# AgamChopra/TorchRegister

Hardware: AMD Instinct MI355X
Metric: registration iterations/sec (3D 256^3 fp32, affine+NCC) (higher is better)
Workload: dtype f32; 1 GPU; 3D 256^3 fp32 affine+NCC, 8 independent pairs per GPU (BASELINE.json configs[3] share of one GPU), ADAM on theta; pairs_per_gpu=8, pairs_total=8, loss=NCC(alpha=100), optimizer=adam, preconditioning=100 untimed iterations before the warm-up (clock settling); value_cold has none, parallelism=1 x independent shards, no collective

## Files before the change

include/trx.h:

```cpp
#ifndef TRX_H
#define TRX_H

#include <stddef.h>
#include <stdint.h>

#ifdef __cplusplus
extern "C" {
#endif

#define TRX_VERSION 240
#define TRX_PSTRIDE 12

typedef enum {
    TRX_OK = 0,
    TRX_ERR_ARG = -1,
    TRX_ERR_NDIM = -2,
    TRX_ERR_WORKSPACE = -3,
    TRX_ERR_HIP = -4,
    TRX_ERR_CAPACITY = -5
} trx_status;

#define TRX_FLAG_GATHER_PATH 1u
#define TRX_FLAG_SINGLE_GEOM 2u
#define TRX_FLAG_TWO_PASS_FLOW 4u
#define TRX_FLAG_DEEP_TILE 8u
#define TRX_FLAG_SAVE_LAST 256u
#define TRX_FLAG_NEAREST 128u
#define TRX_FLAG_NO_ZSTREAM 32u
#define TRX_FLAG_ZSTREAM 64u
#define TRX_FLAG_NO_EFT 512u
#define TRX_FLAG_EFT 1024u
#define TRX_FLAG_ZS_FUSED 2048u
#define TRX_FLAG_WALK_DOWN 8192u
#define TRX_FLAG_NO_PINGPONG 16384u
#define TRX_FLAG_NO_ZS_FLAT 4096u
#define TRX_FLAG_ONE_KERNEL 32768u
#define TRX_FLAG_NO_CARRY 65536u
#define TRX_FLAG_NO_ROT_DEEP_TILE 16u

typedef struct {
    const float *moving;
    const float *target;
    size_t moving_stride;
    size_t target_stride;
    int ndim, B, D, H, W;
    const float *xn, *yn, *zn;
    unsigned flags;
} trx_volumes;

typedef struct {
    float w_mse, w_ncc, ncc_alpha, w_ssd, ssd_alpha;
} trx_loss_cfg;
// ... 150 lines not shown
```

torchregister_amd/_lib.py:

```python
import ctypes
import os

import torch

_HERE = os.path.dirname(os.path.abspath(__file__))
LIB_PATH = os.path.join(_HERE, "lib", "libtrx.so")

PSTRIDE = 12
OPT_SGD, OPT_ADAM = 0, 1
PARAM_AFFINE, PARAM_RIGID = 0, 1
FLAG_GATHER_PATH, FLAG_SINGLE_GEOM, FLAG_TWO_PASS_FLOW, FLAG_DEEP_TILE, FLAG_NO_ROT_DEEP_TILE, FLAG_NO_ZSTREAM, FLAG_ZSTREAM, FLAG_NEAREST, FLAG_SAVE_LAST = 1, 2, 4, 8, 16, 32, 64, 128, 256
FLAG_NO_EFT, FLAG_EFT = 512, 1024
FLAG_WALK_DOWN, FLAG_NO_PINGPONG = 8192, 16384
FLAG_NO_ZS_FLAT = 4096
FLAG_ONE_KERNEL = 32768
FLAG_NO_CARRY = 65536
FLAG_ZS_FUSED = 2048

c_float_p = ctypes.POINTER(ctypes.c_float)
c_int_p = ctypes.POINTER(ctypes.c_int)


class TrxError(RuntimeError):
    pass


class Volumes(ctypes.Structure):
    _fields_ = [("moving", ctypes.c_void_p), ("target", ctypes.c_void_p),
                ("moving_stride", ctypes.c_size_t), ("target_stride", ctypes.c_size_t),
                ("ndim", ctypes.c_int), ("B", ctypes.c_int), ("D", ctypes.c_int), ("H", ctypes.c_int), ("W", ctypes.c_int),
                ("xn", ctypes.c_void_p), ("yn", ctypes.c_void_p), ("zn", ctypes.c_void_p), ("flags", ctypes.c_uint)]
# ... 123 lines not shown
```

torchregister_amd/csrc/affine.hip:

```cpp
#ifdef TRX_DEV
#include <cstdlib>
#endif
#include "trx_dev.h"

#include "trx_common.h"

namespace trx {

struct AffineGeom {
    int TX, TY, logTX, RPT, nxseg, nychunk, nblk;
};

static AffineGeom affine_geom(const trx_volumes &v, int target_blocks_total)
{
    AffineGeom g;
    int tx = 16, l = 4;
    while (tx < v.W && tx < TRX_BLOCK) { tx <<= 1; l++; }
    g.TX = tx; g.logTX = l; g.TY = TRX_BLOCK / tx;
    g.nxseg = (v.W + tx - 1) / tx;
    long rows = (long)v.D * v.H * g.nxseg * v.B;
    long rpt = rows / ((long)g.TY * target_blocks_total);
    if (rpt < 1) rpt = 1;
    if (rpt > 64) rpt = 64;
    g.RPT = (int)rpt;
// ... 1204 lines not shown
    zs_step_main<MODE, 0>(vol, theta, zg, zgf, partials, rows_used, stride, 0, ring);
}

template <int MODE>
__global__ __launch_bounds__(ZS64::Threads, TRX_ZS_MIN_WAVES) void affine_zs_one_kernel(trx_volumes vol, const float *__restrict__ theta, ZGeom zg, ZGeom zgf, float *__restrict__ partials,
                                                                                        int *__restrict__ rows_used, int stride, TileGeom tgR)
{
    constexpr int kAllocZ = ZSF::Alloc > ZS64::Alloc ? ZSF::Alloc : ZS64::Alloc;
    constexpr int kAlloc = GeomR::BoxAlloc > kAllocZ ? GeomR::BoxAlloc : kAllocZ;
    __shared__ __attribute__((aligned(16))) float ring[kAlloc];
    zs_step_main<MODE, 1>(vol, theta, zg, zgf, partials, rows_used, stride, tgR.blocks_per_pair, ring);
}

template <int MODE>
__global__ __launch_bounds__(ECfg::Threads, 4) void affine_eft_step_kernel(trx_volumes vol, const float *__restrict__ theta, TileGeom tg, float *__restrict__ partials,
                                                                           int *__restrict__ rows_used, int stride, int with_d, int with_rd, int zs_planes_)
{
    const bool zs_first = zs_planes_ < 0;
    const int zs_planes = zs_first ? 0 : zs_planes_;
    __shared__ __attribute__((aligned(16))) float lds[ECfg::Alloc];
    __shared__ int s_ef[64];
    const int wave = trx_wave_index(), lane = trx_lane_id();
    const float fD = (float)vol.D, fH = (float)vol.H, fW = (float)vol.W;
    if (stride < 0) {
        if ((int)blockIdx.x >= tg.blocks_per_pair) return;
        const int b = blockIdx.y;
        const float *th = theta + (size_t)b * TRX_PSTRIDE;
        bool take = __builtin_amdgcn_readfirstlane((int)eft_wants(dual_choice(th, fD, fH, fW, with_d != 0, with_rd != 0, zs_planes), th, fD, fH, fW)) &&
                    __builtin_amdgcn_readfirstlane((int)ef_candidate(th, fD, fH, fW));
        if (take) {
            const EfMap m = ef_map(th, fD, fH, fW);
// ... 22 lines not shown
    const bool flat = stride >= 0;
#if TRX_EF_STAMP
    if (flat && wave == 0 && lane == 0) { for (int k = 1; k < 8; k++) trx_ef_blocks[blockIdx.x * 8 + k] = 0; trx_ef_blocks[blockIdx.x * 8] = __builtin_amdgcn_s_memrealtime(); }
#endif
    int pre = 0, total = 1;
    if (flat) {
    if (zs_first && __builtin_amdgcn_readfirstlane(rows_used[vol.B]) == 0) return;
    unsigned long long zs_mask = 0;
    if (zs_first) zs_mask = (unsigned long long)(unsigned)__builtin_amdgcn_readfirstlane(rows_used[vol.B + 1]) | ((unsigned long long)(unsigned)__builtin_amdgcn_readfirstlane(rows_used[vol.B + 2]) << 32);
    const bool free_l = lane < vol.B && !((zs_mask >> lane) & 1ull);
    const bool cand_l = free_l && eft_wants(dual_choice(theta + (size_t)lane * TRX_PSTRIDE, fD, fH, fW, with_d != 0, with_rd != 0, zs_planes),
                                                  theta + (size_t)lane * TRX_PSTRIDE, fD, fH, fW) &&
                        ef_candidate(theta + (size_t)lane * TRX_PSTRIDE, fD, fH, fW);
    const unsigned long long cand = __builtin_amdgcn_ballot_w64(cand_l);
    unsigned long long fit = 0;
    if (cand) {
        if (wave == 0) s_ef[lane] = 0;
        __syncthreads();
        unsigned long long rest = cand;
        for (int k = 0; rest; k++) {
            const int pb = __builtin_ctzll(rest);
            rest &= rest - 1;
            if ((k & (ECfg::Waves - 1)) != wave) continue;
            const EfMap m = ef_map(theta + (size_t)pb * TRX_PSTRIDE, fD, fH, fW);
            const EfDims d = ef_dims(m);
            const int g = ef_plan_granules_wave(m, d, lane);
            if (lane == 0) s_ef[pb] = (d.ok && g > 0 && g <= ECfg::GCap) ? 1 : 0;
        }
        __syncthreads();
        fit = __builtin_amdgcn_ballot_w64(s_ef[lane] != 0) & cand;
    }
// ... 23 lines not shown
        if (flat) {
            if (tickets) {
                int ord = qk / per_pair_q;
                const int j = qk - ord * per_pair_q;
                if (vol.flags & TRX_FLAG_WALK_DOWN) ord = total / tg.blocks_per_pair - 1 - ord;
                pair = __builtin_popcountll(__builtin_amdgcn_ballot_w64(pre <= ord * tg.blocks_per_pair));
                v = q + 8 * j;
            } else {
                pair = __builtin_popcountll(__builtin_amdgcn_ballot_w64(pre <= item));
                const int off = pair > 0 ? __builtin_amdgcn_readlane(pre, pair - 1) : 0;
                v = (item - off + 104 * pair) % tg.blocks_per_pair;
            }
        }
        v = __builtin_amdgcn_readfirstlane(v); pair = __builtin_amdgcn_readfirstlane(pair);
        if (item != it0) __syncthreads();
        eft_body<MODE>(vol, theta, tg, partials, lds, v, pair, rows_stride, wave, pr, pair != planned);
        planned = pair;
#if TRX_EF_STAMP
        if (flat && wave == 0 && lane == 0) { trx_ef_blocks[blockIdx.x * 8 + 1 + min((item - it0) / it_step, 5)] = __builtin_amdgcn_s_memrealtime(); }
#endif
        if (tickets) {
            if (wave == 0 && lane == 0) {
                const int first = (int)gridDim.x >> 3;
                int nq = blockIdx.x & 7, k = qlen;
                for (int t = 0; t < 8 && k >= qlen; t++) {
                    nq = ((int)blockIdx.x + t) & 7;
                    k = __hip_atomic_fetch_add(rows_used + vol.B + 3 + nq, 1, __ATOMIC_RELAXED, __HIP_MEMORY_SCOPE_AGENT) + first;
                }
                s_ef[63] = k < qlen ? ((nq << 24) | k) : -1;
            }
            __syncthreads();
            const int nx = __builtin_amdgcn_readfirstlane(s_ef[63]);
            if (nx < 0) break;
            q = nx >> 24; qk = nx & 0xffffff;
        }
    }
}

#pragma clang diagnostic pop


__global__ void fill_tables_kernel(float *__restrict__ tab, int W, int H, int D)
{
    const int i = blockIdx.x * blockDim.x + threadIdx.x;
    if (i < W) tab[i] = (float)(2 * i + 1) / (float)W - 1.0f;
    if (i < H) tab[W + i] = (float)(2 * i + 1) / (float)H - 1.0f;
    if (i < D) tab[W + H + i] = (float)(2 * i + 1) / (float)D - 1.0f;
}

struct LossCoef {
    double total, mse, ncc, ssd, cy, cw, c0;
};

// ... 206 lines not shown
    }
    if (i < NT) {
        if (theta_out) theta_out[i] = th_new;
        if (theta_lds) theta_lds[i] = th_new;
    }
}

constexpr int kCarryStride = 64;
constexpr int kCarryTheta = 0, kCarryParam = 12, kCarryM = 24, kCarryV = 36, kCarryStep = 48;

template <int ND>
__global__ __launch_bounds__(TRX_FIN_THREADS) void affine_finalize_kernel(const float *__restrict__ partials, int nblk,
                                                                          double nvox, int D, int H, int W,
                                                                          trx_loss_cfg lc, trx_opt_cfg oc,
                                                                          trx_affine_state st, const int *__restrict__ rows_used = nullptr, int mse_rows = 0,
                                                                          const float *__restrict__ state_in = nullptr)
{
    constexpr int NP = np_full(ND);
    constexpr int NT = ND * (ND + 1);
    constexpr int NPOSE = (ND == 3) ? 6 : 3;
    __shared__ double S[64];
    const int b = blockIdx.x;
    __shared__ double sh_dth[NT];
    __shared__ float sh_pose[NPOSE];
    const int i = threadIdx.x;
    const bool rigid = st.mode == TRX_PARAM_RIGID;
    float *param = st.param + (size_t)b * TRX_PSTRIDE;
    float *theta = st.theta + (size_t)b * TRX_PSTRIDE;
    FinRegs<ND> r;
    if (i < 64) {
        if (state_in) {
            const float *sb = state_in + (size_t)b * kCarryStride;
            r = fin_load<ND>(sb + kCarryParam, sb + kCarryTheta, sb + kCarryM, sb + kCarryV, reinterpret_cast<const int *>(sb + kCarryStep), st.best_loss + b,
                             oc.kind == TRX_OPT_ADAM, rigid, i);
        } else {
            r = fin_load<ND>(param, theta, st.adam_m ? st.adam_m + (size_t)b * TRX_PSTRIDE : nullptr, st.adam_v ? st.adam_v + (size_t)b * TRX_PSTRIDE : nullptr, st.step + b,
                             st.best_loss + b, oc.kind == TRX_OPT_ADAM, rigid, i);
        }
    }
    {
        int rows = nblk;
        if (rows_used) rows = min(abs(rows_used[b]) & kRowsMask, nblk);
        if (ND == 3 && mse_rows) reduce_partials<kNpMse>(partials + (size_t)b * nblk * kNpMse, rows, S);
        else reduce_partials<NP>(partials + (size_t)b * nblk * NP, rows, S);
    }
    if (i >= 64) return;
    fin_apply<ND>(S, r, b, i, nvox, D, H, W, lc, oc, st, mse_rows, param, theta, st.adam_m ? st.adam_m + (size_t)b * TRX_PSTRIDE : nullptr,
                  st.adam_v ? st.adam_v + (size_t)b * TRX_PSTRIDE : nullptr, st.step + b, true, nullptr, sh_dth, sh_pose);
}

template <int MODE>
__device__ __forceinline__ void carry_prologue(CarryKPtr c, int b, bool designated, int D, int H, int W, float *scratch, float *s_th, int wave, int lane)
{
    constexpr int NP = (MODE == 4) ? kNpMse : np_full(3);
    constexpr int NT = 12;
    const float *prev = c->prev_partials;
    const float *sp = c->state_prev;
    float *sn = c->state_next;
    const trx_affine_state st = {c->st.mode, c->st.param, c->st.theta, c->st.adam_m, c->st.adam_v, c->st.best_theta, c->st.best_loss, c->st.best_idx, c->st.losses,
                                 c->st.losses_capacity, c->st.step, c->st.grad};
    const trx_opt_cfg oc = {c->oc.kind, c->oc.lr, c->oc.beta1, c->oc.beta2, c->oc.eps};
    const bool adam = oc.kind == TRX_OPT_ADAM, rigid = st.mode == TRX_PARAM_RIGID;
    const float *src_theta = sp ? sp + (size_t)b * kCarryStride + kCarryTheta : st.theta + (size_t)b * TRX_PSTRIDE;
// ... 362 lines not shown
    int dev = 0, cus = 0;
    if (hipGetDevice(&dev) != hipSuccess || hipDeviceGetAttribute(&cus, hipDeviceAttributeMultiprocessorCount, dev) != hipSuccess || cus <= 0)
        return TRX_PERSISTENT_BLOCKS;
    return 2 * cus;
}

enum DualInstance { kTwoBody = 3, kFiveBody = 0, kBehindZs = 4, kCarry = 6 };
template <int W> struct Which { static constexpr int value = W; };
struct F1Plan {
    TileGeom ta, tr, td, trd, tef;
    ZGeom zg, zgf;
    int rows, slots;
    bool flat;
    bool zs_first, one_kernel;
    int eft;
    DualInstance dual;
};

static F1Plan f1_candidates(const trx_volumes &v)
{
    F1Plan p = F1Plan{};
    p.ta = tile_geom<GeomA>(v); p.tr = tile_geom<GeomR>(v); p.td = tile_geom<GeomD>(v); p.trd = p.tef = tile_geom<GeomRD>(v);
    if (zs_shape_ok<ZS64>(v)) p.zg = zs_geom<ZS64>(v);
    if (zs_shape_ok<ZSF>(v)) p.zgf = zs_geom<ZSF>(v);
    return p;
}

static int f1_rows(const F1Plan &p)
{
    return max(max(max(p.ta.blocks_per_pair, p.tr.blocks_per_pair), max(p.td.blocks_per_pair, p.trd.blocks_per_pair)),
// ... 19 lines not shown
    else if (p.zg.blocks_per_pair > 0 && !(v.flags & TRX_FLAG_ZSTREAM)) {
        const long zb = (long)p.zg.blocks_per_pair * v.B;
        if (zb < TRX_ZS_MIN_BLOCKS || p.zg.planes_per_seg < TRX_ZS_MIN_PLANES) p.zg = ZGeom{};
        else if (zb > slots / 2 && zb < slots && (long)p.ta.blocks_per_pair * v.B <= slots) p.zg = ZGeom{};
    }
    if (p.zg.blocks_per_pair == 0) p.zgf = ZGeom{};
    const TileGeom tef = p.tef;
    p.tef = TileGeom{};
    p.rows = f1_rows(p);
    p.flat = v.B <= 64 && (long)p.rows * v.B >= 2 * slots;
    const bool eft_sizes = (long)v.H * v.W * 4 < (1l << 24) && (size_t)v.D * v.H * v.W < ((size_t)1 << 29);
    if (tef.tiles_per_seg <= 64 && eft_sizes && !(v.flags & TRX_FLAG_NO_EFT) && (p.flat || (v.flags & TRX_FLAG_EFT))) {
        p.tef = tef;
        p.eft = tef.blocks_per_pair;
        p.rows = f1_rows(p);
    }
    if (v.flags & TRX_FLAG_NO_ZS_FLAT) p.zgf = ZGeom{};
    p.zs_first = p.flat && p.zg.blocks_per_pair > 0 && !(v.flags & TRX_FLAG_ZS_FUSED);
    p.one_kernel = p.zs_first && (v.flags & TRX_FLAG_ONE_KERNEL);
    const bool two_body = !p.flat && p.td.blocks_per_pair == 0 && p.trd.blocks_per_pair == 0 && p.zg.blocks_per_pair == 0 && p.eft == 0;
    p.dual = p.zs_first ? kBehindZs : !two_body ? kFiveBody : carry ? kCarry : kTwoBody;
    return p;
}

struct AffineWs {
    size_t rows, off_tab, off_rows_used, off_part2, off_rows_used2, off_carry, bytes;
};
static AffineWs affine_ws(const trx_volumes &v)
{
    AffineWs w;
    AffineGeom g = affine_geom(v, kTargetBlocks);
    w.rows = (size_t)g.nblk;
    if (v.ndim == 3) w.rows = max(w.rows, (size_t)f1_rows(f1_candidates(v)));
    w.off_tab = ((size_t)v.B * w.rows * np_full(3) * sizeof(float) + 255) & ~(size_t)255;
    w.off_rows_used = w.off_tab + (((size_t)(v.W + v.H + v.D) * sizeof(float) + 255) & ~(size_t)255);
    const size_t notes = ((size_t)(v.B + 11) * sizeof(int) + 255) & ~(size_t)255;
    w.off_part2 = w.off_rows_used + notes;
    w.off_rows_used2 = w.off_part2 + (v.ndim == 3 ? w.off_tab : 0);
    w.off_carry = w.off_rows_used2 + (v.ndim == 3 ? notes : 0);
    w.bytes = w.off_carry + (v.ndim == 3 ? (((size_t)2 * v.B * kCarryStride * sizeof(float) + 255) & ~(size_t)255) : 0);
    return w;
}

extern "C" size_t trx_affine_workspace_bytes(const trx_volumes *vol)
{
    if (check_vol(vol, false) != TRX_OK) return 0;
    return affine_ws(*vol).bytes;
}

extern "C" size_t trx_affine_workspace_rows_offset(const trx_volumes *vol)
{
    if (check_vol(vol, false) != TRX_OK) return 0;
    return affine_ws(*vol).off_rows_used;
}

// ... 1 lines not shown
{
    if (check_vol(vol, false) != TRX_OK || !theta_host || vol->ndim != 3) return 0;
    const F1Plan p = f1_plan(*vol, persistent_blocks(), true, false);
    if (p.zg.blocks_per_pair == 0) return 0;
    const float fD = (float)vol->D, fH = (float)vol->H, fW = (float)vol->W;
    for (int b = 0; b < vol->B; b++) {
        const float *th = theta_host + (size_t)b * TRX_PSTRIDE;
        if (zs_nsub<ZS64>(th, fD, fH, fW, p.zg.planes_per_seg) > 0) continue;
        if (p.zgf.blocks_per_pair > 0 && zs_nsub<ZSF>(th, fD, fH, fW, p.zgf.planes_per_seg) > 0) continue;
        return 0;
    }
    return 1;
}

static bool use_tile_path(const trx_volumes *vol) { return vol->ndim == 3 && !(vol->flags & TRX_FLAG_GATHER_PATH); }

struct CarryLaunch {
    int parity;
    CarryKArgs args;
    bool used;
    float *partials_out;
};

template <int MODE>
static int launch_accum(const trx_volumes *vol, const float *theta, const AffineGeom &g, int channels, size_t chan_stride,
                        float *partials, hipStream_t s)
{
    dim3 grid(g.nblk, vol->B), block(TRX_BLOCK);
    if (vol->ndim == 3)
        hipLaunchKernelGGL((affine_accum_kernel<3, MODE>), grid, block, 0, s, *vol, theta, g, channels, chan_stride, partials);
// ... 9 lines not shown
{
    const dim3 grid = p.flat ? dim3(p.slots, 1) : dim3(p.rows, v.B * channels);
    const int zero_surplus = rows_used == nullptr, rows_stride = p.flat ? p.rows : 0;
    auto launch = [&](auto which, auto... carry_args) {
        hipLaunchKernelGGL((affine_tile_dual_kernel<MODE, decltype(which)::value>), grid, dim3(512), 0, s, v, theta, p.ta, p.tr, channels, out, zero_surplus, p.td, p.trd, p.zg,
                           rows_used, rows_stride, p.eft, carry_args...);
    };
    if constexpr (MODE == 0 || MODE == 4)
        if (p.dual == kCarry) return launch(Which<kCarry>{}, *carry);
    if constexpr (MODE == 0 || MODE == 1 || MODE == 4)
        if (p.dual == kBehindZs) return launch(Which<kBehindZs>{});
    p.dual == kTwoBody ? launch(Which<kTwoBody>{}) : launch(Which<kFiveBody>{});
}

template <int MODE>
static int launch_f1(const trx_volumes *vol, const float *theta, float *partials, int *nblk, hipStream_t s, const int **rows_used = nullptr, CarryLaunch *cl = nullptr)
{
    if (rows_used) *rows_used = nullptr;
    if (cl) cl->used = false;
    if (!use_tile_path(vol)) {
        if constexpr (MODE == 4) return TRX_ERR_ARG;
        else {
            AffineGeom g = affine_geom(*vol, kTargetBlocks);
            *nblk = g.nblk;
            return launch_accum<MODE>(vol, theta, g, 1, 0, partials, s);
        }
    }
    trx_volumes v = *vol;
    const AffineWs ws = affine_ws(*vol);
    float *const ws_base = partials;
    const bool odd = cl != nullptr && cl->parity != 0;
// ... 4 lines not shown
        const int n = max(v.W, max(v.H, v.D));
        hipLaunchKernelGGL(fill_tables_kernel, dim3((n + 255) / 256), dim3(256), 0, s, tab, v.W, v.H, v.D);
        TRX_CHECK_LAUNCH();
        v.xn = tab; v.yn = tab + v.W; v.zn = tab + v.W + v.H;
    }
    if (!use_dual(vol)) {
        const TileGeom t = tile_geom(*vol);
        hipLaunchKernelGGL((affine_tile_kernel<MODE>), dim3(t.blocks_per_pair, vol->B), dim3(kTileThreads), 0, s, v, theta, t, 1, partials);
        TRX_CHECK_LAUNCH();
        *nblk = t.blocks_per_pair;
        return TRX_OK;
    }
    int *const ru = rows_used ? (int *)((char *)ws_base + (odd ? ws.off_rows_used2 : ws.off_rows_used)) : nullptr;
    const F1Plan p = f1_plan(*vol, persistent_blocks(), ru != nullptr && (MODE == 0 || MODE == 4), cl != nullptr);
    if constexpr (MODE == 0 || MODE == 4) {
        if (p.one_kernel) hipLaunchKernelGGL((affine_zs_one_kernel<MODE>), dim3(p.slots, 1), dim3(ZS64::Threads), 0, s, v, theta, p.zg, p.zgf, partials, ru, p.rows, p.tr);
        else {
            if (p.zs_first) {
                hipLaunchKernelGGL((affine_zs_step_kernel<MODE>), dim3(p.slots, 1), dim3(ZS64::Threads), 0, s, v, theta, p.zg, p.zgf, partials, ru, p.rows);
                TRX_CHECK_LAUNCH();
            }
            if (p.eft) {
                const int wd = p.td.blocks_per_pair > 0, wrd = p.trd.blocks_per_pair > 0, zp = p.zs_first ? -1 : (p.zg.blocks_per_pair > 0 ? p.zg.planes_per_seg : 0);
                if (p.flat) hipLaunchKernelGGL((affine_eft_step_kernel<MODE>), dim3(p.slots, 1), dim3(ECfg::Threads), 0, s, v, theta, p.tef, partials, ru, p.rows, wd, wrd, zp);
                else hipLaunchKernelGGL((affine_eft_step_kernel<MODE>), dim3(p.tef.blocks_per_pair, vol->B), dim3(ECfg::Threads), 0, s, v, theta, p.tef, partials, ru, -p.rows, wd, wrd, zp);
                TRX_CHECK_LAUNCH();
            }
        }
    }
    if (!p.one_kernel) launch_dual<MODE>(p, s, v, theta, 1, partials, ru, cl ? &cl->args : nullptr);
    TRX_CHECK_LAUNCH();
    if (cl) cl->used = p.dual == kCarry;
    *nblk = p.rows;
    if (rows_used) *rows_used = ru;
    return TRX_OK;
}

static int launch_finalize(const trx_volumes *vol, const trx_loss_cfg *loss, const trx_opt_cfg *opt, const trx_affine_state *st, const float *partials, int nblk,
                           const int *rows_used, bool mse_only, const float *state_in, hipStream_t s)
{
    const double nvox = (double)vol->D * vol->H * vol->W;
    if (vol->ndim == 3)
        hipLaunchKernelGGL((affine_finalize_kernel<3>), dim3(vol->B), dim3(TRX_FIN_THREADS), 0, s, partials, nblk, nvox,
                           vol->D, vol->H, vol->W, *loss, *opt, *st, rows_used, mse_only ? 1 : 0, state_in);
    else
        hipLaunchKernelGGL((affine_finalize_kernel<2>), dim3(vol->B), dim3(TRX_FIN_THREADS), 0, s, partials, nblk, nvox,
                           vol->D, vol->H, vol->W, *loss, *opt, *st);
    TRX_CHECK_LAUNCH();
    return TRX_OK;
}

static int check_step_args(const trx_volumes *vol, const trx_loss_cfg *loss, const trx_opt_cfg *opt, const trx_affine_state *st, const void *workspace, size_t workspace_bytes)
{
    int rc = check_vol(vol, true);
    if (rc) return rc;
    if (!loss || !opt || !st || !workspace) return TRX_ERR_ARG;
    if (!st->param || !st->theta || !st->best_theta || !st->best_loss || !st->best_idx || !st->step) return TRX_ERR_ARG;
    if (opt->kind != TRX_OPT_SGD && opt->kind != TRX_OPT_ADAM) return TRX_ERR_ARG;
    if (opt->kind == TRX_OPT_ADAM && (!st->adam_m || !st->adam_v)) return TRX_ERR_ARG;
    if (st->mode != TRX_PARAM_AFFINE && st->mode != TRX_PARAM_RIGID) return TRX_ERR_ARG;
    if (workspace_bytes < trx_affine_workspace_bytes(vol)) return TRX_ERR_WORKSPACE;
    return TRX_OK;
}

static bool step_mse_only(const trx_volumes *vol, const trx_loss_cfg *loss) { return (loss->w_ncc == 0.f) && use_tile_path(vol); }

template <class... Args>
static int launch_step_f1(bool mse_only, Args... args) { return mse_only ? launch_f1<4>(args...) : launch_f1<0>(args...); }

static unsigned iteration_flags(const trx_volumes *vol, int k) { return ((k & 1) && !(vol->flags & TRX_FLAG_NO_PINGPONG)) ? vol->flags ^ TRX_FLAG_WALK_DOWN : vol->flags; }

extern "C" int trx_affine_step(const trx_volumes *vol, const trx_loss_cfg *loss, const trx_opt_cfg *opt,
                               const trx_affine_state *st, void *workspace, size_t workspace_bytes, void *stream)
{
    int rc = check_step_args(vol, loss, opt, st, workspace, workspace_bytes);
    if (rc) return rc;
    hipStream_t s = (hipStream_t)stream;
    float *partials = (float *)workspace;
    int nblk = 0;
    const int *rows_used = nullptr;
    const bool mse_only = step_mse_only(vol, loss);
    rc = launch_step_f1(mse_only, vol, st->theta, partials, &nblk, s, &rows_used);
    if (rc) return rc;
    return launch_finalize(vol, loss, opt, st, partials, nblk, rows_used, mse_only, nullptr, s);
}

extern "C" int trx_affine_accumulate(const trx_volumes *vol, const float *theta, void *workspace, size_t workspace_bytes, void *stream)
{
    int rc = check_vol(vol, true);
    if (rc) return rc;
    if (!theta || !workspace) return TRX_ERR_ARG;
    if (workspace_bytes < trx_affine_workspace_bytes(vol)) return TRX_ERR_WORKSPACE;
    int nblk = 0;
    const int *rows_used = nullptr;
    return launch_f1<0>(vol, theta, (float *)workspace, &nblk, (hipStream_t)stream, &rows_used);
}

extern "C" int trx_affine_run(const trx_volumes *vol, const trx_loss_cfg *loss, const trx_opt_cfg *opt,
                              const trx_affine_state *st, int iters, void *workspace, size_t workspace_bytes, void *stream)
// ... 21 lines not shown
            const int *notes = nullptr;
            int rc = launch_step_f1(mse_only, &v, st->theta, base, &nblk, s, &notes, &cl);
            if (rc) return rc;
            if (!cl.used) {
                rc = launch_finalize(vol, loss, opt, st, cl.partials_out, nblk, notes, mse_only, nullptr, s);
                if (rc) return rc;
                first = 1;
                prev_partials = nullptr;
                break;
            }
            prev_partials = cl.partials_out; prev_notes = notes; prev_nblk = nblk;
        }
        if (prev_partials != nullptr)
            return launch_finalize(vol, loss, opt, st, prev_partials, prev_nblk, prev_notes, mse_only, carry_buf, s);
    }
    for (int i = first; i < iters; i++) {
        v.flags = iteration_flags(vol, i);
        int rc = trx_affine_step(&v, loss, opt, st, workspace, workspace_bytes, stream);
        if (rc) return rc;
    }
    return TRX_OK;
}

extern "C" int trx_affine_loss(const trx_volumes *vol, const trx_loss_cfg *loss, const float *theta, float *terms,
                               void *workspace, size_t workspace_bytes, void *stream)
{
    int rc = check_vol(vol, true);
    if (rc) return rc;
    if (!loss || !theta || !terms || !workspace) return TRX_ERR_ARG;
    if (workspace_bytes < trx_affine_workspace_bytes(vol)) return TRX_ERR_WORKSPACE;
    hipStream_t s = (hipStream_t)stream;
    float *partials = (float *)workspace;
    int nblk = 0;
// ... 193 lines not shown
```

torchregister_amd/csrc/affine_eft.h:

```cpp

#ifndef TRX_EF_DBG
#define TRX_EF_DBG 0
#endif
#ifndef TRX_EF_STAMP
#define TRX_EF_STAMP 0
#endif
#if TRX_EF_STAMP
__device__ unsigned long long trx_ef_stamps2[1024 * 8 * 8];
#define TRX_EF_ST2(k) do { if (trx_lane_id() == 0) trx_ef_stamps2[((size_t)((by * rows_stride + bx) & 1023) * 8 + wave) * 8 + (k)] = __builtin_amdgcn_s_memtime() - ef_t0; } while (0)
__device__ unsigned long long trx_ef_blocks[1024 * 8];
__device__ unsigned long long trx_ef_stamps[1024 * 8 * 8];
#endif
#if !TRX_EF_STAMP
#define TRX_EF_ST2(k) do { } while (0)
#endif
#ifndef TRX_EF_EPS
#define TRX_EF_EPS 0.05f
#endif

struct ECfg {
    static constexpr int TX = 16, TY = 16, TZ = 16, Threads = 512, Waves = 8, NH = 2, Rows = 8;
    static constexpr int K = 5;
    static constexpr int NY = 32, NZ = 32;
    static constexpr int TP = 40;
// ... 94 lines not shown

#pragma clang diagnostic push
#pragma clang diagnostic ignored "-Winline-asm"
#pragma clang diagnostic ignored "-Wint-to-pointer-cast"
__device__ __forceinline__ int wave_scan_incl(int v)
{
    v += __builtin_amdgcn_update_dpp(0, v, 0x111, 0xf, 0xf, false);
    v += __builtin_amdgcn_update_dpp(0, v, 0x112, 0xf, 0xf, false);
    v += __builtin_amdgcn_update_dpp(0, v, 0x114, 0xf, 0xf, false);
    v += __builtin_amdgcn_update_dpp(0, v, 0x118, 0xf, 0xf, false);
    v += __builtin_amdgcn_update_dpp(0, v, 0x142, 0xa, 0xf, false);
    v += __builtin_amdgcn_update_dpp(0, v, 0x143, 0xc, 0xf, false);
    return v;
}

struct EfPlanRegs {
    int G, ok;
    int geo[ECfg::K];
    unsigned goff[ECfg::K];
};
template <int MODE>
__device__ __forceinline__ void eft_body(const trx_volumes &vol, const float *__restrict__ theta, const TileGeom &tg, float *__restrict__ partials,
                                         float *lds, const int bx, const int by, const int rows_stride, const int wave_in, EfPlanRegs &pr, const bool replan)
{
    static_assert(MODE == 0 || MODE == 1 || MODE == 4, "step kernels and the moments pass");
    using C = ECfg;
    constexpr int NQ = (MODE == 0) ? 3 : (MODE == 4 ? 1 : 0);
    constexpr int NP = (MODE == 0) ? np_full(3) : (MODE == 4 ? kNpMse : 5);
    constexpr bool kGrad = MODE != 1;
    constexpr int kRows = C::Rows, K = C::K;
    const int b = by;
    const int D = vol.D, H = vol.H, W = vol.W;
    const float *__restrict__ th = uni_ptr(theta + (size_t)b * TRX_PSTRIDE);
    const float *__restrict__ mov = uni_ptr(vol.moving + (size_t)b * vol.moving_stride);
    const float *__restrict__ tgt = uni_ptr(vol.target + (size_t)b * vol.target_stride);
    const float *__restrict__ xtab = uni_ptr(vol.xn), *__restrict__ ytab = uni_ptr(vol.yn), *__restrict__ ztab = uni_ptr(vol.zn);
    const int lane = trx_lane_id();
    const int wave = __builtin_amdgcn_readfirstlane(wave_in);
// ... 13 lines not shown
    const int colx = col % tg.ntx, colz = col / tg.ntx;
    const int X0 = colx * C::TX, Z0 = colz * C::TZ;
    const int nx = min(C::TX, W - X0), nz = min(C::TZ, D - Z0);
    const bool act = (lx < nx) && (lz < nz);
    const int x = X0 + (act ? lx : 0), z = Z0 + (act ? lz : 0);
    const float xn = xtab[x], zn = ztab[z];
    const float base_x = unnorm<3>(xn, fW) + hW * fmaf(t00 - 1.0f, xn, fmaf(t02, zn, t03));
    const float base_y = hH * fmaf(t10, xn, fmaf(t12, zn, t13));
    const float base_z = unnorm<3>(zn, fD) + hD * fmaf(t20, xn, fmaf(t22 - 1.0f, zn, t23));
    const float cxn = xtab[X0], czn = ztab[Z0];
    const float corner_x = uni(unnorm<3>(cxn, fW) + hW * fmaf(t00 - 1.0f, cxn, fmaf(t02, czn, t03)));
    const float corner_y = uni(hH * fmaf(t10, cxn, fmaf(t12, czn, t13)));
    const float corner_z = uni(unnorm<3>(czn, fD) + hD * fmaf(t20, cxn, fmaf(t22 - 1.0f, czn, t23)));
    const int ty_begin = yseg * tg.tiles_per_seg, ty_end = min((yseg + 1) * tg.tiles_per_seg, tg.nty);

    const EfMap mp = ef_map(th, fD, fH, fW);
    const EfDims dm = ef_dims(mp);
    int *ilds = reinterpret_cast<int *>(lds);
    int *tab = ilds + 2 * C::BufFloats;
    int *desc = ilds + C::BufFloats;
    int *wtot = ilds;
    const unsigned lds0 = (unsigned)(uintptr_t)lds;
#if TRX_EF_STAMP
    unsigned long long ef_stamp[6] = {0, 0, 0, 0, 0, 0}, ef_issue[2] = {0, 0};
    const unsigned long long ef_t0 = __builtin_amdgcn_s_memtime();
#endif
    int w4_s, hw4_s;
    asm("s_mov_b32 %0, %1" : "=s"(w4_s) : "s"(W * 4));
    asm("s_mov_b32 %0, %1" : "=s"(hw4_s) : "s"(H * W * 4));
    int *org = ilds + 2 * C::BufFloats + C::TabInts;
    auto lane_origins = [&](int ty_first) {
        if (wave != 0) return;
// ... 1 lines not shown
        const float yn0 = ytab[ty * C::TY], yid0 = unnorm<3>(yn0, fH);
        const float cx = fmaf(sx, yn0, corner_x), cy = yid0 + fmaf(sy, yn0, corner_y), cz = fmaf(sz, yn0, corner_z);
        const bool sane = (fabsf(cx) < 1.0e6f) && (fabsf(cy) < 1.0e6f) && (fabsf(cz) < 1.0e6f);
        const int rx = sane ? (int)floorf(cx) : -100000, ry = sane ? (int)floorf(cy) : -100000, rz = sane ? (int)floorf(cz) : -100000;
        const int x0 = rx + dm.xmin, y0 = ry + dm.dy0, z0 = rz + dm.dz0;
        const bool interior = (x0 >= 0) && (rx + dm.xmax + 3 < W) && (y0 >= 0) && (y0 + dm.ny <= H) && (z0 >= 0) && (z0 + dm.nz <= D);
        const bool outside = (rx + dm.xmax < 0) || (x0 >= W) || (y0 + dm.ny <= 0) || (y0 >= H) || (z0 + dm.nz <= 0) || (z0 >= D);
        int4 v;
        v.x = rx; v.y = ry; v.z = rz;
        v.w = outside ? 0 : (int)((((long long)z0 * H + y0) * W + x0) * 4);
        *reinterpret_cast<int4 *>(org + lane * 8) = v;
        org[lane * 8 + 4] = (interior ? 1 : 0) | (outside ? 2 : 0);
    };
    if (dm.ok) lane_origins(ty_begin);
    if (replan) {
    int cnt_r[2], wlo_r[2], pre_r[2];
#pragma unroll
    for (int h = 0; h < 2; h++) {
        const int r = tid + h * C::Threads, iy = r & (C::NY - 1), iz = r >> 5;
        cnt_r[h] = 0; wlo_r[h] = 0;
        if (dm.ok && iy < dm.ny && iz < dm.nz) cnt_r[h] = ef_row_window(mp, dm.dy0 + iy, dm.dz0 + iz, wlo_r[h]);
        const int p = wave_scan_incl(cnt_r[h]);
        pre_r[h] = p;
        if (lane == 63) wtot[h * C::Waves + wave] = p;
    }
    TRX_EF_ST2(0);
    __syncthreads();
    TRX_EF_ST2(1);
    int G = 0;
    {
        int before[2] = {0, 0};
#pragma unroll
        for (int c = 0; c < 2 * C::Waves; c++) {
            const int t = wtot[c];
            if (c < wave) before[0] += t;
            if (c < C::Waves + wave) before[1] += t;
            G += t;
        }
        pre_r[0] += before[0] - cnt_r[0];
        pre_r[1] += before[1] - cnt_r[1];
    }
    G = __builtin_amdgcn_readfirstlane(G);
    const bool plan_ok = dm.ok && G <= C::GCap && G > 0;
    __syncthreads();
    TRX_EF_ST2(2);
    if (plan_ok) {
#pragma unroll
        for (int h = 0; h < 2; h++) {
            const int r = tid + h * C::Threads, iy = r & (C::NY - 1), iz = r >> 5;
            tab[iz * C::TP + iy] = (pre_r[h] * 4 - wlo_r[h]) * 4;
            for (int k = 0; k < cnt_r[h]; k++) desc[pre_r[h] + k] = (iz << 20) | (iy << 12) | ((wlo_r[h] + 4 * k - dm.xmin) << 2);
        }
    }
    __syncthreads();
    TRX_EF_ST2(3);
#pragma unroll
    for (int k = 0; k < K; k++) {
        const int g = tid + k * C::Threads;
        pr.geo[k] = (plan_ok && g < G) ? desc[g] : 0;
    }
    auto goff_of = [&](int pk) -> unsigned {
        unsigned t0, t1, t2;
        asm("v_and_b32 %0, 0xffc, %1" : "=v"(t0) : "v"(pk));
        asm("v_bfe_u32 %0, %1, 12, 8" : "=v"(t1) : "v"(pk));
        asm("v_mad_u32_u24 %0, %1, %2, %3" : "=v"(t2) : "v"(t1), "s"(w4_s), "v"(t0));
        asm("v_lshrrev_b32 %0, 20, %1" : "=v"(t1) : "v"(pk));
        asm("v_mad_u32_u24 %0, %1, %2, %3" : "=v"(t0) : "v"(t1), "s"(hw4_s), "v"(t2));
        return t0;
    };
#pragma unroll
    for (int k = 0; k < K; k++) pr.goff[k] = goff_of(pr.geo[k]);
    pr.G = G; pr.ok = plan_ok ? 1 : 0;
    __syncthreads();
    TRX_EF_ST2(4);
    }
    const int G = __builtin_amdgcn_readfirstlane(pr.G);
    const bool plan_ok = __builtin_amdgcn_readfirstlane(pr.ok) != 0;
    const int (&geo)[K] = pr.geo;
    const unsigned (&goff)[K] = pr.goff;
#if TRX_EF_STAMP
    ef_stamp[3] = __builtin_amdgcn_s_memtime() - ef_t0;
#endif

    F1Acc acc;
#pragma unroll
    for (int q = 0; q < 3; q++)
#pragma unroll
        for (int c = 0; c < 3; c++) acc.AB[q][c] = (f2)(0.f);
// ... 332 lines not shown
```

Baseline: 26720 pair-iterations/s.

## Precompute EFT gather plans once per pair and publish them to global memory

Moves construction of the per-pair EFT row-window plan (table, descriptors, dims) out of every EFT block into a per-pair publish step. The plan is written to a new workspace region either by the previous iteration's finalize kernel (after the theta update) or by a small standalone plan kernel. EFT blocks then load the plan from global memory instead of rebuilding it with scans and barriers. This removes redundant per-block planning and LDS syncs, at the cost of extra finalize work, an extra kernel launch on the first iteration, and more global traffic.

Result: no change. 26720 pair-iterations/s (median of 2 runs) (+0.0%).

```diff
diff --git a/include/trx.h b/include/trx.h
--- a/include/trx.h
+++ b/include/trx.h
@@ -36,6 +36,7 @@
 #define TRX_FLAG_NO_ZS_FLAT 4096u
 #define TRX_FLAG_ONE_KERNEL 32768u
 #define TRX_FLAG_NO_CARRY 65536u
+#define TRX_FLAG_EFT_BLOCK_PLAN 131072u
 #define TRX_FLAG_NO_ROT_DEEP_TILE 16u
 
 typedef struct {
diff --git a/torchregister_amd/_lib.py b/torchregister_amd/_lib.py
--- a/torchregister_amd/_lib.py
+++ b/torchregister_amd/_lib.py
@@ -15,6 +15,7 @@
 FLAG_NO_ZS_FLAT = 4096
 FLAG_ONE_KERNEL = 32768
 FLAG_NO_CARRY = 65536
+FLAG_EFT_BLOCK_PLAN = 131072
 FLAG_ZS_FUSED = 2048
 
 c_float_p = ctypes.POINTER(ctypes.c_float)
diff --git a/torchregister_amd/csrc/affine.hip b/torchregister_amd/csrc/affine.hip
--- a/torchregister_amd/csrc/affine.hip
+++ b/torchregister_amd/csrc/affine.hip
@@ -1242,7 +1242,8 @@
 
 template <int MODE>
 __global__ __launch_bounds__(ECfg::Threads, 4) void affine_eft_step_kernel(trx_volumes vol, const float *__restrict__ theta, TileGeom tg, float *__restrict__ partials,
-                                                                           int *__restrict__ rows_used, int stride, int with_d, int with_rd, int zs_planes_)
+                                                                           int *__restrict__ rows_used, int stride, int with_d, int with_rd, int zs_planes_,
+                                                                           const int *__restrict__ pub = nullptr)
 {
     const bool zs_first = zs_planes_ < 0;
     const int zs_planes = zs_first ? 0 : zs_planes_;
@@ -1295,7 +1296,9 @@
                         ef_candidate(theta + (size_t)lane * TRX_PSTRIDE, fD, fH, fW);
     const unsigned long long cand = __builtin_amdgcn_ballot_w64(cand_l);
     unsigned long long fit = 0;
-    if (cand) {
+    if (pub) {
+        fit = __builtin_amdgcn_ballot_w64(cand_l && pub[(size_t)min(lane, vol.B - 1) * EfPub::Stride + EfPub::Fit] != 0);
+    } else if (cand) {
         if (wave == 0) s_ef[lane] = 0;
         __syncthreads();
         unsigned long long rest = cand;
@@ -1349,7 +1352,7 @@
         }
         v = __builtin_amdgcn_readfirstlane(v); pair = __builtin_amdgcn_readfirstlane(pair);
         if (item != it0) __syncthreads();
-        eft_body<MODE>(vol, theta, tg, partials, lds, v, pair, rows_stride, wave, pr, pair != planned);
+        eft_body<MODE>(vol, theta, tg, partials, lds, v, pair, rows_stride, wave, pr, pair != planned, pub);
         planned = pair;
 #if TRX_EF_STAMP
         if (flat && wave == 0 && lane == 0) { trx_ef_blocks[blockIdx.x * 8 + 1 + min((item - it0) / it_step, 5)] = __builtin_amdgcn_s_memrealtime(); }
@@ -1372,6 +1375,30 @@
     }
 }
 
+struct EfPlanArgs {
+    int *pub;
+    int with_d, with_rd, zs_planes;
+    int zg_planes, zgf_planes;
+};
+__device__ __forceinline__ bool eft_offered(const float *th, float fD, float fH, float fW, const EfPlanArgs &a)
+{
+    if (a.zs_planes < 0) {
+        if (zs_nsub<ZS64>(th, fD, fH, fW, a.zg_planes) > 0) return false;
+        if (a.zgf_planes > 0 && zs_nsub<ZSF>(th, fD, fH, fW, a.zgf_planes) > 0) return false;
+    }
+    return eft_wants(dual_choice(th, fD, fH, fW, a.with_d != 0, a.with_rd != 0, max(a.zs_planes, 0)), th, fD, fH, fW) && ef_candidate(th, fD, fH, fW);
+}
+constexpr int kEfPlanLds = ECfg::TabInts + ECfg::GCap + 16;
+__global__ __launch_bounds__(ECfg::Threads) void eft_plan_kernel(const float *__restrict__ theta, int D, int H, int W, EfPlanArgs ep)
+{
+    __shared__ __attribute__((aligned(16))) int s_plan[kEfPlanLds];
+    const int b = blockIdx.x;
+    const float *th = uni_ptr(theta + (size_t)b * TRX_PSTRIDE);
+    const float fD = (float)D, fH = (float)H, fW = (float)W;
+    const bool cand = __builtin_amdgcn_readfirstlane((int)eft_offered(th, fD, fH, fW, ep)) != 0;
+    ef_plan_publish(th, fD, fH, fW, cand, ep.pub + (size_t)b * EfPub::Stride, s_plan, threadIdx.x);
+}
+
 #pragma clang diagnostic pop
 
 
@@ -1608,12 +1635,13 @@
                                                                           double nvox, int D, int H, int W,
                                                                           trx_loss_cfg lc, trx_opt_cfg oc,
                                                                           trx_affine_state st, const int *__restrict__ rows_used = nullptr, int mse_rows = 0,
-                                                                          const float *__restrict__ state_in = nullptr)
+                                                                          const float *__restrict__ state_in = nullptr, EfPlanArgs ep = EfPlanArgs{})
 {
     constexpr int NP = np_full(ND);
     constexpr int NT = ND * (ND + 1);
     constexpr int NPOSE = (ND == 3) ? 6 : 3;
     __shared__ double S[64];
+    __shared__ float s_th[NT];
     const int b = blockIdx.x;
     __shared__ double sh_dth[NT];
     __shared__ float sh_pose[NPOSE];
@@ -1638,9 +1666,20 @@
         if (ND == 3 && mse_rows) reduce_partials<kNpMse>(partials + (size_t)b * nblk * kNpMse, rows, S);
         else reduce_partials<NP>(partials + (size_t)b * nblk * NP, rows, S);
     }
-    if (i >= 64) return;
-    fin_apply<ND>(S, r, b, i, nvox, D, H, W, lc, oc, st, mse_rows, param, theta, st.adam_m ? st.adam_m + (size_t)b * TRX_PSTRIDE : nullptr,
-                  st.adam_v ? st.adam_v + (size_t)b * TRX_PSTRIDE : nullptr, st.step + b, true, nullptr, sh_dth, sh_pose);
+    if (i < 64)
+        fin_apply<ND>(S, r, b, i, nvox, D, H, W, lc, oc, st, mse_rows, param, theta, st.adam_m ? st.adam_m + (size_t)b * TRX_PSTRIDE : nullptr,
+                      st.adam_v ? st.adam_v + (size_t)b * TRX_PSTRIDE : nullptr, st.step + b, true, (ND == 3 && ep.pub) ? s_th : nullptr, sh_dth, sh_pose);
+    if constexpr (ND == 3) {
+        if (ep.pub == nullptr || i >= ECfg::Threads) return;
+        __shared__ __attribute__((aligned(16))) int s_plan[kEfPlanLds];
+        __syncthreads();
+        float th[NT];
+#pragma unroll
+        for (int k = 0; k < NT; k++) th[k] = s_th[k];
+        const float fD = (float)D, fH = (float)H, fW = (float)W;
+        const bool cand = __builtin_amdgcn_readfirstlane((int)eft_offered(th, fD, fH, fW, ep)) != 0;
+        ef_plan_publish(th, fD, fH, fW, cand, ep.pub + (size_t)b * EfPub::Stride, s_plan, i);
+    }
 }
 
 template <int MODE>
@@ -2033,6 +2072,7 @@
     bool flat;
     bool zs_first, one_kernel;
     int eft;
+    bool eft_plan;
     DualInstance dual;
 };
 
@@ -2082,6 +2122,7 @@
         p.tef = tef;
         p.eft = tef.blocks_per_pair;
         p.rows = f1_rows(p);
+        p.eft_plan = p.flat && !(v.flags & TRX_FLAG_EFT_BLOCK_PLAN);
     }
     if (v.flags & TRX_FLAG_NO_ZS_FLAT) p.zgf = ZGeom{};
     p.zs_first = p.flat && p.zg.blocks_per_pair > 0 && !(v.flags & TRX_FLAG_ZS_FUSED);
@@ -2092,7 +2133,7 @@
 }
 
 struct AffineWs {
-    size_t rows, off_tab, off_rows_used, off_part2, off_rows_used2, off_carry, bytes;
+    size_t rows, off_tab, off_rows_used, off_part2, off_rows_used2, off_carry, off_plan, bytes;
 };
 static AffineWs affine_ws(const trx_volumes &v)
 {
@@ -2106,7 +2147,8 @@
     w.off_part2 = w.off_rows_used + notes;
     w.off_rows_used2 = w.off_part2 + (v.ndim == 3 ? w.off_tab : 0);
     w.off_carry = w.off_rows_used2 + (v.ndim == 3 ? notes : 0);
-    w.bytes = w.off_carry + (v.ndim == 3 ? (((size_t)2 * v.B * kCarryStride * sizeof(float) + 255) & ~(size_t)255) : 0);
+    w.off_plan = w.off_carry + (v.ndim == 3 ? (((size_t)2 * v.B * kCarryStride * sizeof(float) + 255) & ~(size_t)255) : 0);
+    w.bytes = w.off_plan + (v.ndim == 3 ? (size_t)v.B * EfPub::Stride * sizeof(int) : 0);
     return w;
 }
 
@@ -2138,6 +2180,14 @@
 }
 
 static bool use_tile_path(const trx_volumes *vol) { return vol->ndim == 3 && !(vol->flags & TRX_FLAG_GATHER_PATH); }
+
+static EfPlanArgs eft_plan_args(const F1Plan &p, void *ws_base, const AffineWs &ws)
+{
+    if (!p.eft_plan) return EfPlanArgs{};
+    return EfPlanArgs{(int *)((char *)ws_base + ws.off_plan), p.td.blocks_per_pair > 0, p.trd.blocks_per_pair > 0,
+                      p.zs_first ? -1 : (p.zg.blocks_per_pair > 0 ? p.zg.planes_per_seg : 0),
+                      p.zg.planes_per_seg, p.zgf.blocks_per_pair > 0 ? p.zgf.planes_per_seg : 0};
+}
 
 struct CarryLaunch {
     int parity;
@@ -2177,7 +2227,8 @@
 }
 
 template <int MODE>
-static int launch_f1(const trx_volumes *vol, const float *theta, float *partials, int *nblk, hipStream_t s, const int **rows_used = nullptr, CarryLaunch *cl = nullptr)
+static int launch_f1(const trx_volumes *vol, const float *theta, float *partials, int *nblk, hipStream_t s, const int **rows_used = nullptr, CarryLaunch *cl = nullptr,
+                     bool plans_published = false)
 {
     if (rows_used) *rows_used = nullptr;
     if (cl) cl->used = false;
@@ -2212,6 +2263,11 @@
     int *const ru = rows_used ? (int *)((char *)ws_base + (odd ? ws.off_rows_used2 : ws.off_rows_used)) : nullptr;
     const F1Plan p = f1_plan(*vol, persistent_blocks(), ru != nullptr && (MODE == 0 || MODE == 4), cl != nullptr);
     if constexpr (MODE == 0 || MODE == 4) {
+        const EfPlanArgs ep = p.one_kernel ? EfPlanArgs{} : eft_plan_args(p, ws_base, ws);
+        if (ep.pub && !plans_published) {
+            hipLaunchKernelGGL(eft_plan_kernel, dim3(vol->B), dim3(ECfg::Threads), 0, s, theta, v.D, v.H, v.W, ep);
+            TRX_CHECK_LAUNCH();
+        }
         if (p.one_kernel) hipLaunchKernelGGL((affine_zs_one_kernel<MODE>), dim3(p.slots, 1), dim3(ZS64::Threads), 0, s, v, theta, p.zg, p.zgf, partials, ru, p.rows, p.tr);
         else {
             if (p.zs_first) {
@@ -2220,7 +2276,7 @@
             }
             if (p.eft) {
                 const int wd = p.td.blocks_per_pair > 0, wrd = p.trd.blocks_per_pair > 0, zp = p.zs_first ? -1 : (p.zg.blocks_per_pair > 0 ? p.zg.planes_per_seg : 0);
-                if (p.flat) hipLaunchKernelGGL((affine_eft_step_kernel<MODE>), dim3(p.slots, 1), dim3(ECfg::Threads), 0, s, v, theta, p.tef, partials, ru, p.rows, wd, wrd, zp);
+                if (p.flat) hipLaunchKernelGGL((affine_eft_step_kernel<MODE>), dim3(p.slots, 1), dim3(ECfg::Threads), 0, s, v, theta, p.tef, partials, ru, p.rows, wd, wrd, zp, (const int *)ep.pub);
                 else hipLaunchKernelGGL((affine_eft_step_kernel<MODE>), dim3(p.tef.blocks_per_pair, vol->B), dim3(ECfg::Threads), 0, s, v, theta, p.tef, partials, ru, -p.rows, wd, wrd, zp);
                 TRX_CHECK_LAUNCH();
             }
@@ -2235,12 +2291,18 @@
 }
 
 static int launch_finalize(const trx_volumes *vol, const trx_loss_cfg *loss, const trx_opt_cfg *opt, const trx_affine_state *st, const float *partials, int nblk,
-                           const int *rows_used, bool mse_only, const float *state_in, hipStream_t s)
+                           const int *rows_used, bool mse_only, const float *state_in, hipStream_t s, void *publish_ws = nullptr, bool *published = nullptr)
 {
     const double nvox = (double)vol->D * vol->H * vol->W;
+    EfPlanArgs ep = EfPlanArgs{};
+    if (publish_ws && use_tile_path(vol) && use_dual(vol)) {
+        const F1Plan p = f1_plan(*vol, persistent_blocks(), true, false);
+        if (!p.one_kernel) ep = eft_plan_args(p, publish_ws, affine_ws(*vol));
+    }
+    if (published) *published = ep.pub != nullptr;
     if (vol->ndim == 3)
         hipLaunchKernelGGL((affine_finalize_kernel<3>), dim3(vol->B), dim3(TRX_FIN_THREADS), 0, s, partials, nblk, nvox,
-                           vol->D, vol->H, vol->W, *loss, *opt, *st, rows_used, mse_only ? 1 : 0, state_in);
+                           vol->D, vol->H, vol->W, *loss, *opt, *st, rows_used, mse_only ? 1 : 0, state_in, ep);
     else
         hipLaunchKernelGGL((affine_finalize_kernel<2>), dim3(vol->B), dim3(TRX_FIN_THREADS), 0, s, partials, nblk, nvox,
                            vol->D, vol->H, vol->W, *loss, *opt, *st);
@@ -2268,8 +2330,8 @@
 
 static unsigned iteration_flags(const trx_volumes *vol, int k) { return ((k & 1) && !(vol->flags & TRX_FLAG_NO_PINGPONG)) ? vol->flags ^ TRX_FLAG_WALK_DOWN : vol->flags; }
 
-extern "C" int trx_affine_step(const trx_volumes *vol, const trx_loss_cfg *loss, const trx_opt_cfg *opt,
-                               const trx_affine_state *st, void *workspace, size_t workspace_bytes, void *stream)
+static int affine_step(const trx_volumes *vol, const trx_loss_cfg *loss, const trx_opt_cfg *opt, const trx_affine_state *st, void *workspace, size_t workspace_bytes,
+                       void *stream, bool *plans_published, bool publish_next)
 {
     int rc = check_step_args(vol, loss, opt, st, workspace, workspace_bytes);
     if (rc) return rc;
@@ -2278,9 +2340,16 @@
     int nblk = 0;
     const int *rows_used = nullptr;
     const bool mse_only = step_mse_only(vol, loss);
-    rc = launch_step_f1(mse_only, vol, st->theta, partials, &nblk, s, &rows_used);
+    rc = launch_step_f1(mse_only, vol, st->theta, partials, &nblk, s, &rows_used, (CarryLaunch *)nullptr, *plans_published);
     if (rc) return rc;
-    return launch_finalize(vol, loss, opt, st, partials, nblk, rows_used, mse_only, nullptr, s);
+    return launch_finalize(vol, loss, opt, st, partials, nblk, rows_used, mse_only, nullptr, s, publish_next ? workspace : nullptr, plans_published);
+}
+
+extern "C" int trx_affine_step(const trx_volumes *vol, const trx_loss_cfg *loss, const trx_opt_cfg *opt,
+                               const trx_affine_state *st, void *workspace, size_t workspace_bytes, void *stream)
+{
+    bool plans_published = false;
+    return affine_step(vol, loss, opt, st, workspace, workspace_bytes, stream, &plans_published, false);
 }
 
 extern "C" int trx_affine_accumulate(const trx_volumes *vol, const float *theta, void *workspace, size_t workspace_bytes, void *stream)
@@ -2332,9 +2401,10 @@
         if (prev_partials != nullptr)
             return launch_finalize(vol, loss, opt, st, prev_partials, prev_nblk, prev_notes, mse_only, carry_buf, s);
     }
+    bool plans_published = false;
     for (int i = first; i < iters; i++) {
         v.flags = iteration_flags(vol, i);
-        int rc = trx_affine_step(&v, loss, opt, st, workspace, workspace_bytes, stream);
+        int rc = affine_step(&v, loss, opt, st, workspace, workspace_bytes, stream, &plans_published, i + 1 < iters);
         if (rc) return rc;
     }
     return TRX_OK;
diff --git a/torchregister_amd/csrc/affine_eft.h b/torchregister_amd/csrc/affine_eft.h
--- a/torchregister_amd/csrc/affine_eft.h
+++ b/torchregister_amd/csrc/affine_eft.h
@@ -132,6 +132,88 @@
     return v;
 }
 
+template <class Stamp>
+__device__ __forceinline__ bool ef_plan_build(const EfMap &mp, const EfDims &dm, int *wtot, int *tab, int *desc, const int tid, const int wave, const int lane, int &G_out,
+                                              Stamp &&stamp)
+{
+    using C = ECfg;
+    int cnt_r[2], wlo_r[2], pre_r[2];
+#pragma unroll
+    for (int h = 0; h < 2; h++) {
+        const int r = tid + h * C::Threads, iy = r & (C::NY - 1), iz = r >> 5;
+        cnt_r[h] = 0; wlo_r[h] = 0;
+        if (dm.ok && iy < dm.ny && iz < dm.nz) cnt_r[h] = ef_row_window(mp, dm.dy0 + iy, dm.dz0 + iz, wlo_r[h]);
+        const int p = wave_scan_incl(cnt_r[h]);
+        pre_r[h] = p;
+        if (lane == 63) wtot[h * C::Waves + wave] = p;
+    }
+    stamp(0);
+    __syncthreads();
+    stamp(1);
+    int G = 0;
+    {
+        int before[2] = {0, 0};
+#pragma unroll
+        for (int c = 0; c < 2 * C::Waves; c++) {
+            const int t = wtot[c];
+            if (c < wave) before[0] += t;
+            if (c < C::Waves + wave) before[1] += t;
+            G += t;
+        }
+        pre_r[0] += before[0] - cnt_r[0];
+        pre_r[1] += before[1] - cnt_r[1];
+    }
+    G = __builtin_amdgcn_readfirstlane(G);
+    const bool plan_ok = dm.ok && G <= C::GCap && G > 0;
+    __syncthreads();
+    stamp(2);
+    if (plan_ok) {
+#pragma unroll
+        for (int h = 0; h < 2; h++) {
+            const int r = tid + h * C::Threads, iy = r & (C::NY - 1), iz = r >> 5;
+            tab[iz * C::TP + iy] = (pre_r[h] * 4 - wlo_r[h]) * 4;
+            for (int k = 0; k < cnt_r[h]; k++) desc[pre_r[h] + k] = (iz << 20) | (iy << 12) | ((wlo_r[h] + 4 * k - dm.xmin) << 2);
+        }
+    }
+    __syncthreads();
+    stamp(3);
+    G_out = G;
+    return plan_ok;
+}
+
+struct EfPub {
+    static constexpr int Fit = 0, G = 1, Dims = 2, Tab = 16, Geo = Tab + ECfg::TabInts, Ints = Geo + ECfg::K * ECfg::Threads;
+    static constexpr int Stride = (Ints + 63) & ~63;
+    static_assert(ECfg::TabInts % 4 == 0 && ECfg::TabInts / 4 <= ECfg::Threads && Tab % 4 == 0, "the table travels as 16-byte pieces, one per thread");
+};
+__device__ __forceinline__ void ef_plan_publish(const float *th, float fD, float fH, float fW, bool cand, int *__restrict__ pub, int *lds, const int tid)
+{
+    using C = ECfg;
+    if (!cand) {
+        if (tid == 0) pub[EfPub::Fit] = 0;
+        return;
+    }
+    const int wave = __builtin_amdgcn_readfirstlane(tid >> 6), lane = tid & 63;
+    int *tab = lds, *desc = lds + C::TabInts, *wtot = desc + C::GCap;
+    for (int i = tid; i < C::TabInts; i += C::Threads) tab[i] = 0;
+    const EfMap mp = ef_map(th, fD, fH, fW);
+    const EfDims dm = ef_dims(mp);
+    int G;
+    const bool ok = ef_plan_build(mp, dm, wtot, tab, desc, tid, wave, lane, G, [](int) {});
+    if (tid == 0) {
+        pub[EfPub::Fit] = ok ? 1 : 0; pub[EfPub::G] = G;
+        pub[EfPub::Dims + 0] = dm.dy0; pub[EfPub::Dims + 1] = dm.dz0; pub[EfPub::Dims + 2] = dm.ny; pub[EfPub::Dims + 3] = dm.nz;
+        pub[EfPub::Dims + 4] = dm.xmin; pub[EfPub::Dims + 5] = dm.xmax;
+    }
+    if (!ok) return;
+    if (tid < C::TabInts / 4) reinterpret_cast<int4 *>(pub + EfPub::Tab)[tid] = reinterpret_cast<const int4 *>(tab)[tid];
+#pragma unroll
+    for (int k = 0; k < C::K; k++) {
+        const int g = tid + k * C::Threads;
+        pub[EfPub::Geo + g] = g < G ? desc[g] : 0;
+    }
+}
+
 struct EfPlanRegs {
     int G, ok;
     int geo[ECfg::K];
@@ -139,7 +221,8 @@
 };
 template <int MODE>
 __device__ __forceinline__ void eft_body(const trx_volumes &vol, const float *__restrict__ theta, const TileGeom &tg, float *__restrict__ partials,
-                                         float *lds, const int bx, const int by, const int rows_stride, const int wave_in, EfPlanRegs &pr, const bool replan)
+                                         float *lds, const int bx, const int by, const int rows_stride, const int wave_in, EfPlanRegs &pr, const bool replan,
+                                         const int *__restrict__ pub = nullptr)
 {
     static_assert(MODE == 0 || MODE == 1 || MODE == 4, "step kernels and the moments pass");
     using C = ECfg;
@@ -183,8 +266,17 @@
     const float corner_z = uni(unnorm<3>(czn, fD) + hD * fmaf(t20, cxn, fmaf(t22 - 1.0f, czn, t23)));
     const int ty_begin = yseg * tg.tiles_per_seg, ty_end = min((yseg + 1) * tg.tiles_per_seg, tg.nty);
 
-    const EfMap mp = ef_map(th, fD, fH, fW);
-    const EfDims dm = ef_dims(mp);
+    EfMap mp;
+    EfDims dm;
+    if (pub) {
+        pub = uni_ptr(pub + (size_t)b * EfPub::Stride);
+        dm.dy0 = pub[EfPub::Dims + 0]; dm.dz0 = pub[EfPub::Dims + 1]; dm.ny = pub[EfPub::Dims + 2]; dm.nz = pub[EfPub::Dims + 3];
+        dm.xmin = pub[EfPub::Dims + 4]; dm.xmax = pub[EfPub::Dims + 5];
+        dm.ok = pub[EfPub::Fit] != 0;
+    } else {
+        mp = ef_map(th, fD, fH, fW);
+        dm = ef_dims(mp);
+    }
     int *ilds = reinterpret_cast<int *>(lds);
     int *tab = ilds + 2 * C::BufFloats;
     int *desc = ilds + C::BufFloats;
@@ -216,50 +308,20 @@
     };
     if (dm.ok) lane_origins(ty_begin);
     if (replan) {
-    int cnt_r[2], wlo_r[2], pre_r[2];
-#pragma unroll
-    for (int h = 0; h < 2; h++) {
-        const int r = tid + h * C::Threads, iy = r & (C::NY - 1), iz = r >> 5;
-        cnt_r[h] = 0; wlo_r[h] = 0;
-        if (dm.ok && iy < dm.ny && iz < dm.nz) cnt_r[h] = ef_row_window(mp, dm.dy0 + iy, dm.dz0 + iz, wlo_r[h]);
-        const int p = wave_scan_incl(cnt_r[h]);
-        pre_r[h] = p;
-        if (lane == 63) wtot[h * C::Waves + wave] = p;
-    }
-    TRX_EF_ST2(0);
-    __syncthreads();
-    TRX_EF_ST2(1);
     int G = 0;
-    {
-        int before[2] = {0, 0};
-#pragma unroll
-        for (int c = 0; c < 2 * C::Waves; c++) {
-            const int t = wtot[c];
-            if (c < wave) before[0] += t;
-            if (c < C::Waves + wave) before[1] += t;
-            G += t;
-        }
-        pre_r[0] += before[0] - cnt_r[0];
-        pre_r[1] += before[1] - cnt_r[1];
-    }
-    G = __builtin_amdgcn_readfirstlane(G);
-    const bool plan_ok = dm.ok && G <= C::GCap && G > 0;
-    __syncthreads();
-    TRX_EF_ST2(2);
-    if (plan_ok) {
-#pragma unroll
-        for (int h = 0; h < 2; h++) {
-            const int r = tid + h * C::Threads, iy = r & (C::NY - 1), iz = r >> 5;
-            tab[iz * C::TP + iy] = (pre_r[h] * 4 - wlo_r[h]) * 4;
-            for (int k = 0; k < cnt_r[h]; k++) desc[pre_r[h] + k] = (iz << 20) | (iy << 12) | ((wlo_r[h] + 4 * k - dm.xmin) << 2);
-        }
-    }
-    __syncthreads();
-    TRX_EF_ST2(3);
+    bool plan_ok;
+    if (pub) {
+        G = __builtin_amdgcn_readfirstlane(pub[EfPub::G]);
+        plan_ok = dm.ok;
+        if (plan_ok && tid < C::TabInts / 4) reinterpret_cast<int4 *>(tab)[tid] = reinterpret_cast<const int4 *>(pub + EfPub::Tab)[tid];
+    } else {
+        plan_ok = ef_plan_build(mp, dm, wtot, tab, desc, tid, wave, lane, G, [&](int k) { TRX_EF_ST2(k); });
+    }
 #pragma unroll
     for (int k = 0; k < K; k++) {
         const int g = tid + k * C::Threads;
-        pr.geo[k] = (plan_ok && g < G) ? desc[g] : 0;
+        if (pub) pr.geo[k] = plan_ok ? pub[EfPub::Geo + g] : 0;
+        else pr.geo[k] = (plan_ok && g < G) ? desc[g] : 0;
     }
     auto goff_of = [&](int pk) -> unsigned {
         unsigned t0, t1, t2;
@@ -273,7 +335,7 @@
 #pragma unroll
     for (int k = 0; k < K; k++) pr.goff[k] = goff_of(pr.geo[k]);
     pr.G = G; pr.ok = plan_ok ? 1 : 0;
-    __syncthreads();
+    if (!pub) __syncthreads();
     TRX_EF_ST2(4);
     }
     const int G = __builtin_amdgcn_readfirstlane(pr.G);
```
